# matajoh/fourier_feature_nets

Measured on AMD Instinct MI355X. Metric: rays/sec (train), higher is better.
Workload: dtype f32

## Files before the change

### fourier_feature_nets_amd/csrc/wgrad_common.h

```cpp
#pragma once
#include "common.h"

namespace ffn {

typedef float f32x4 __attribute__((ext_vector_type(4)));
typedef float f32x16 __attribute__((ext_vector_type(16)));

constexpr int kPartialFloats = 16 * 16 * 64 + 256;

__host__ __device__ __forceinline__ constexpr int ffn_wgrad_fold(int n_quads) {
    return n_quads <= 8 ? 4 : (n_quads <= 16 ? 2 : 1);
}

__device__ __forceinline__ f32x4 zero4() { f32x4 z; z[0] = z[1] = z[2] = z[3] = 0.0f; return z; }

template <typename T>
__device__ __forceinline__ T* uniform_ptr(T* p) {
    const uint64_t v = reinterpret_cast<uint64_t>(p);
    const uint32_t lo = __builtin_amdgcn_readfirstlane((uint32_t)v);
    const uint32_t hi = __builtin_amdgcn_readfirstlane((uint32_t)(v >> 32));
    return reinterpret_cast<T*>(((uint64_t)hi << 32) | lo);
}

constexpr int kImageBytes = 32 * 1024;
constexpr int kImageStride = kImageBytes + 512;
constexpr int kUnitLdsBytes = 4 * kImageStride;
__device__ __forceinline__ constexpr int image_a(int cur) { return cur * kImageStride; }
__device__ __forceinline__ constexpr int image_b(int cur) { return (2 + cur) * kImageStride; }

__device__ __forceinline__ void head_segment(const ffn_mlp_chain& ch, const ffn_wgrad_unit& unit,
                                             const ffn_wgrad_segment& seg, char* smem,
                                             const float* __restrict__ saved,
                                             const float* __restrict__ d_logits, int64_t n,
                                             int64_t num_blocks, float* __restrict__ partials) {
    const int tid = threadIdx.x;
    const int lane = tid & 63;
    const int sb = lane >> 2;
    const int li = lane & 3;
    const int wave = __builtin_amdgcn_readfirstlane(tid >> 6);
    const int lg_col = unit.m_slot, lg_n = unit.m_cq0;
    const bool col_ok = li < lg_n;
    const int64_t x_stride = (int64_t)ch.slot_channels[unit.n_slot] * 128;
    const char* x_s = reinterpret_cast<const char*>(saved + ch.slot_offset[unit.n_slot] * num_blocks * 32) +
                      unit.n_cq0 * 512 + seg.blk_begin * x_stride;
    x_s = uniform_ptr(x_s);
    const int c_last = (unit.n_quads >> 3) - 1;
    const int t16 = tid * 16;
    f32x4 acc[16];
#pragma unroll
    for (int q = 0; q < 16; ++q) acc[q] = zero4();
    float bsum = 0.0f;
    const int dl_lane = 4 * sb + (col_ok ? lg_col + li : 0);
    auto load_dl = [&](int64_t blk, float (&dst)[2]) {
        typedef const float __attribute__((address_space(1)))* gfloat;
        if ((blk + 1) * 32 <= n) {
            gfloat base = (gfloat)uniform_ptr(d_logits + blk * 128);
#pragma unroll
            for (int hs = 0; hs < 2; ++hs) {
                const float v = base[dl_lane + 64 * hs];
                dst[hs] = col_ok ? v : 0.0f;
            }
        } else {
#pragma unroll
            for (int hs = 0; hs < 2; ++hs) {
                const int64_t sample = blk * 32 + 16 * hs + sb;
                const int64_t sc = sample < n ? sample : n - 1;
                const float v = d_logits[sc * 4 + (col_ok ? lg_col + li : 0)];
                dst[hs] = (col_ok && sample < n) ? v : 0.0f;
            }
        }
    };
    f32x4 R[8];
    typedef const f32x4 __attribute__((address_space(1)))* gptr;
#define FFN_REQUEST(j)                                                                         \
    do {                                                                                       \
        gptr chunk = (gptr)(x_s + ((j) < c_last ? (j) : c_last) * 4096);                       \
        asm volatile("" : "+s"(chunk));                                                        \
        R[j] = __builtin_nontemporal_load(&chunk[tid]);                                                                     \
    } while (0)
#define FFN_DEPOSIT(cur, j) *reinterpret_cast<f32x4*>(smem + image_a(cur) + (j) * 4096 + t16) = R[j]
    float dl[2], dl_next[2];
    load_dl(seg.blk_begin, dl);
#pragma unroll
    for (int j = 0; j < 8; ++j) FFN_REQUEST(j);
#pragma unroll
    for (int j = 0; j < 8; ++j) FFN_DEPOSIT(0, j);
    x_s += x_stride;
    if (seg.blk_begin + 1 < seg.blk_end) {
#pragma unroll
        for (int j = 0; j < 8; ++j) FFN_REQUEST(j);
    }
    x_s += x_stride;
    asm volatile("s_waitcnt lgkmcnt(0)" ::: "memory");
    __builtin_amdgcn_s_barrier();
    unsigned a_at[16];
#pragma unroll
    for (int q = 0; q < 16; ++q) {
        const int quad = 16 * wave + q;
        a_at[q] = quad < unit.n_quads ? (unsigned)(quad * 512 + ((sb ^ q) << 4) + 4 * li)
                                      : (unsigned)(kImageBytes + 4 * li);
    }
    for (int64_t blk = seg.blk_begin; blk < seg.blk_end; ++blk) {
        const int cur = (int)((blk - seg.blk_begin) & 1);
        const bool has1 = blk + 1 < seg.blk_end, has2 = blk + 2 < seg.blk_end;
        load_dl(has1 ? blk + 1 : blk, dl_next);
        const char* img = smem + image_a(cur);
        bsum += dl[0] + dl[1];
#pragma unroll
        for (int q = 0; q < 16; ++q) {
            const float a0 = *reinterpret_cast<const float*>(img + a_at[q]);
            const float a1 = *reinterpret_cast<const float*>(img + a_at[q] + 256);
            acc[q] = __builtin_amdgcn_mfma_f32_4x4x1f32(a0, dl[0], acc[q], 0, 0, 0);
            acc[q] = __builtin_amdgcn_mfma_f32_4x4x1f32(a1, dl[1], acc[q], 0, 0, 0);
            if (q < 8) {
                if (q < 2) {
                    if (has1) {
#pragma unroll
                        for (int jj = 0; jj < 4; ++jj) FFN_DEPOSIT(cur ^ 1, q * 4 + jj);
                    }
                } else if (q < 6) {
                    if (has2) {
#pragma unroll
                        for (int jj = 0; jj < 2; ++jj) FFN_REQUEST((q - 2) * 2 + jj);
                    }
                }
            }
        }
        x_s += x_stride;
        asm volatile("s_waitcnt lgkmcnt(0)" ::: "memory");
        __builtin_amdgcn_s_barrier();
        dl[0] = dl_next[0];
        dl[1] = dl_next[1];
    }
#undef FFN_REQUEST
#undef FFN_DEPOSIT
    float* out = partials + (int64_t)(seg.slot + wave) * kPartialFloats;
#pragma unroll
    for (int q = 0; q < 16; ++q)
#pragma unroll
        for (int i = 0; i < 4; ++i) out[(q * 4 + i) * 64 + lane] = acc[q][i];
    out[16 * 16 * 64 + lane] = bsum;
}

}
```

### fourier_feature_nets_amd/mlp_engine.py

```python

import ctypes
import os
from typing import Dict, List, Optional, Sequence

import torch

from . import _lib
from ._lib import c_i, c_i64
from .ops import _call, _dev, _want, _want_numel

MAX_STEPS = 16
BIAS_LDS_FLOATS = 4096
WGRAD_GROUPS = 256
UNIT_COST = {4: 24, 2: 13, 1: 8}
HEAD_COST = 5
FOLD_COST = {(2, 2): 7, (2, 4): 5, (1, 2): 4, (1, 4): 3}
if os.environ.get("FFN_FOLD_COST"):
    _c = [int(v) for v in os.environ["FFN_FOLD_COST"].split(",")]
    FOLD_COST = {(2, 2): _c[0], (2, 4): _c[1], (1, 2): _c[2], (1, 4): _c[3]}
UNIT_COST16 = {4: 24, 2: 24, 1: 20}
HEAD_COST16 = 13
if os.environ.get("FFN_UNIT_COST16"):
    _c = [int(v) for v in os.environ["FFN_UNIT_COST16"].split(",")]
    UNIT_COST16, HEAD_COST16 = {4: _c[0], 2: _c[1], 1: _c[2]}, _c[3]
UNIT_COST_X6 = {4: 24, 2: 17, 1: 17}
HEAD_COST_X6 = 10
if os.environ.get("FFN_UNIT_COST_X6"):
    _c = [int(v) for v in os.environ["FFN_UNIT_COST_X6"].split(",")]
    UNIT_COST_X6, HEAD_COST_X6 = {4: _c[0], 2: _c[1], 1: _c[2]}, _c[3]
if os.environ.get("FFN_UNIT_COST"):
    _c = [int(v) for v in os.environ["FFN_UNIT_COST"].split(",")]
    UNIT_COST, HEAD_COST = {4: _c[0], 2: _c[1], 1: _c[2]}, _c[3]


TAIL_PAIRS = os.environ.get("FFN_TAIL_PAIRS", "1") == "1"
TAIL_QUADS = os.environ.get("FFN_TAIL_QUADS", "1") == "1"
TAIL_MAX_FULL_ROUNDS = 16


class FfnEncoding(ctypes.Structure):
    _fields_ = [("b", ctypes.c_void_p), ("a", ctypes.c_void_p), ("num_freq", ctypes.c_int32),
                ("include_input", ctypes.c_int32), ("scale", ctypes.c_float),
                ("width", ctypes.c_int32)]


class FfnStep(ctypes.Structure):
    _fields_ = [("act_groups", ctypes.c_int32), ("aux_groups", ctypes.c_int32),
                ("enc_id", ctypes.c_int32), ("lg_col", ctypes.c_int32), ("lg_n", ctypes.c_int32),
                ("out_tiles", ctypes.c_int32), ("relu", ctypes.c_int32), ("dst", ctypes.c_int32),
                ("out_col", ctypes.c_int32), ("out_n", ctypes.c_int32),
                ("save_in_slot", ctypes.c_int32), ("save_out_slot", ctypes.c_int32),
                ("mask_slot", ctypes.c_int32), ("save_enc_slot", ctypes.c_int32),
                ("head_off", ctypes.c_int32), ("out_slot", ctypes.c_int32),
                ("w_off", ctypes.c_int64), ("b_off", ctypes.c_int64)]


class FfnMlpChain(ctypes.Structure):
    _fields_ = [("enc", FfnEncoding * 2), ("step", FfnStep * MAX_STEPS),
                ("num_steps", ctypes.c_int32), ("num_slots", ctypes.c_int32),
                ("bias_floats", ctypes.c_int32), ("wide", ctypes.c_int32),
                ("slot_channels", ctypes.c_int32 * MAX_STEPS),
                ("slot_offset", ctypes.c_int64 * MAX_STEPS)]


class FfnWgradUnit(ctypes.Structure):
    _fields_ = [("m_slot", ctypes.c_int32), ("m_cq0", ctypes.c_int32), ("m_quads", ctypes.c_int32),
                ("want_bias", ctypes.c_int32), ("n_slot", ctypes.c_int32), ("n_cq0", ctypes.c_int32),
                ("n_quads", ctypes.c_int32), ("kind", ctypes.c_int32)]


class FfnWgradSegment(ctypes.Structure):
    _fields_ = [("job", ctypes.c_int32), ("slot", ctypes.c_int32),
                ("blk_begin", ctypes.c_int64), ("blk_end", ctypes.c_int64)]


class FfnReduceJob(ctypes.Structure):
    _fields_ = [("kind", ctypes.c_int32), ("slot_begin", ctypes.c_int32),
                ("slot_end", ctypes.c_int32), ("m_ch0", ctypes.c_int32), ("rows", ctypes.c_int32),
                ("n_quad0", ctypes.c_int32), ("n_quads", ctypes.c_int32),
                ("k_base", ctypes.c_int32), ("ld", ctypes.c_int32), ("has_bias", ctypes.c_int32),
                ("lg_n", ctypes.c_int32), ("slot_stride", ctypes.c_int32),
                ("n_fold", ctypes.c_int32), ("reserved", ctypes.c_int32),
                ("w_grad_off", ctypes.c_int64), ("b_grad_off", ctypes.c_int64),
                ("col_map", ctypes.c_void_p)]


class FfnPackJob(ctypes.Structure):
    _fields_ = [("src", ctypes.c_void_p), ("dst", ctypes.c_void_p), ("col_map", ctypes.c_void_p),
                ("kind", ctypes.c_int32), ("rows", ctypes.c_int32), ("cols", ctypes.c_int32),
                ("ld", ctypes.c_int32), ("transpose", ctypes.c_int32), ("groups", ctypes.c_int32),
                ("tiles", ctypes.c_int32), ("dst_rs", ctypes.c_int32), ("dst_cs", ctypes.c_int32),
                ("reserved", ctypes.c_int32)]


class FfnRenderRays(ctypes.Structure):
    _fields_ = [("starts", ctypes.c_void_p), ("directions", ctypes.c_void_p),
                ("near_far", ctypes.c_void_p), ("num_rays_total", ctypes.c_int64),
                ("ray_index", ctypes.c_void_p), ("ray_base", ctypes.c_int64),
                ("valid", ctypes.c_void_p), ("num_rays", ctypes.c_int32),
                ("num_samples", ctypes.c_int32), ("unit", ctypes.c_void_p),
                ("t_values", ctypes.c_void_p)]


class FfnOccupancy(ctypes.Structure):
    _fields_ = [("bits", ctypes.c_void_p), ("box_min", ctypes.c_float * 3),
                ("box_size", ctypes.c_float * 3), ("resolution", ctypes.c_int32)]


class FfnRenderOut(ctypes.Structure):
    _fields_ = [("color", ctypes.c_void_p), ("alpha", ctypes.c_void_p), ("depth", ctypes.c_void_p),
                ("nan_flag", ctypes.c_void_p), ("image", ctypes.c_void_p),
                ("pixel_offset", ctypes.c_int64)]


def _struct_array_to_device(items, device):
    if not items:
        return torch.zeros((0,), dtype=torch.uint8, device=device)
    arr = (type(items[0]) * len(items))(*items)
    host = torch.frombuffer(bytearray(bytes(arr)), dtype=torch.uint8)
    return host.to(device)


class EncodingSpec:

    def __init__(self, b: Optional[torch.Tensor], a: Optional[torch.Tensor], scale: float,
                 include_input: bool, device: Optional[torch.device] = None, num_inputs: int = 3):
        if num_inputs not in (1, 2, 3):
            raise NotImplementedError("encodings of 1, 2 or 3 inputs (got %d)" % num_inputs)
        self.num_inputs = int(num_inputs)
        self.num_freq = 0 if b is None else int(b.shape[1])
        dev = device if device is not None else (b.device if b is not None else None)
        if b is None:
            b = torch.zeros((3, 1), dtype=torch.float32, device=dev)
        elif b.shape[0] != num_inputs:
            raise ValueError("B has %d rows for %d inputs" % (b.shape[0], num_inputs))
        elif num_inputs < 3:
            b = torch.cat([b, torch.zeros((3 - num_inputs, b.shape[1]), dtype=b.dtype,
                                          device=b.device)])
        if a is None:
            a = torch.ones((max(self.num_freq, 1),), dtype=torch.float32, device=dev)
        self.b = b.contiguous()
        self.a = a.contiguous()
        self.scale = float(scale)
        self.include_input = bool(include_input) or self.num_freq == 0
        if self.num_freq > 256:
            raise NotImplementedError("encodings with more than 256 frequencies")
        natural = 2 * self.num_freq + (self.num_inputs if self.include_input else 0)
        self.natural_width = natural
        self.width = ((natural + 31) // 32) * 32

    def natural_index(self, internal: int) -> int:
        freq = self.num_freq
        if internal < 2 * freq:
            k = internal >> 1
            return k if (internal & 1) == 0 else freq + k
        if self.include_input and internal < 2 * freq + self.num_inputs:
            return internal
        return -1


class DenseSpec:

    def __init__(self, weight, bias, act_in: int, enc_id: Optional[int], relu: bool,
                 to_logits: Optional[tuple] = None):
        self.weight = weight
        self.bias = bias
        self.act_in = int(act_in)
        self.enc_id = enc_id
        self.relu = bool(relu)
        self.to_logits = to_logits
        self.out = int(weight.shape[0])
        self.ld = int(weight.shape[1])
        self.out_p = self.out
        self.act_in_p = self.act_in


MAX_HIDDEN_CHANNELS = 1024


def _padded_width(channels: int, wide=False) -> int:
    widths = {0: (32, 64, 128, 256), 1: (64, 128, 256, 512), 3: (128, 256, 512, 1024)}[int(wide)]
    for width in widths:
        if channels <= width:
            return width
    raise NotImplementedError("fused MLP kernels support hidden layers of up to %d channels "
                              "(got %d)" % (MAX_HIDDEN_CHANNELS, channels))


def _tiles(channels: int, wide=False) -> int:
    return _padded_width(channels, wide) // 32


class Workspace:

    def __init__(self, prog: "MlpProgram", n: int):
        self.n = n
        blocks = (n + 31) // 32
        self._dz_floats = prog.dz_channels * 32 * blocks
        self._prog, self._blocks = prog, blocks
        self._plans = {}
        self.partials = None
        self.use_plan("f32")

    @property
    def dz(self) -> torch.Tensor:
        return self._prog._dz_buffer(self._dz_floats)

    def use_plan(self, precision: str):
        plan = self._plans.get(precision)
        if plan is None:
            dev = self._prog.device
            raw = self._prog._plan_wgrad(self._blocks, precision)
            launches = [(kind, _struct_array_to_device(segs, dev), torch.tensor(starts, dtype=torch.int32, device=dev))
                        for kind, segs, starts in raw["launches"]]
            plan = dict(unit_segments=launches[0][1], unit_seg_start=launches[0][2], launches=launches,
                        reduce_jobs=_struct_array_to_device(raw["reduce_jobs"], dev),
                        num_reduce_jobs=len(raw["reduce_jobs"]),
                        partial_floats=raw["slots"] * self._prog.partial_floats)
            self._plans[precision] = plan
        self.unit_segments = plan["unit_segments"]
        self.unit_seg_start = plan["unit_seg_start"]
        self.launches = plan["launches"]
        self.reduce_jobs = plan["reduce_jobs"]
        self.num_reduce_jobs = plan["num_reduce_jobs"]
        if self.partials is None or self.partials.numel() < plan["partial_floats"]:
            self.partials = torch.empty((plan["partial_floats"],), dtype=torch.float32,
                                        device=self._prog.device)


class MlpProgram:

    def __init__(self, encodings: Sequence[EncodingSpec], layers: Sequence[DenseSpec],
                 device: torch.device, planning_only: bool = False):
        if device.type != "cuda" and not planning_only:
            raise RuntimeError("MlpProgram needs a GPU device; there is no CPU fallback")
        if len(layers) > MAX_STEPS:
            raise NotImplementedError("at most %d dense layers" % MAX_STEPS)
        self.partial_floats = 16 * 16 * 64 + 256
        if not planning_only:
            lib = _lib.load()
            lib.ffn_mlp_wgrad_partial_floats.restype = ctypes.c_int64
            assert int(lib.ffn_mlp_wgrad_partial_floats()) == self.partial_floats
        self.device = device
        self.encodings = list(encodings)
        self.layers = list(layers)
        self.uses_views = any(spec.enc_id == 1 for spec in self.layers)
        self._workspaces: Dict[int, Workspace] = {}
        self._build_forward()
        self._build_backward()
        self._build_wgrad_jobs()
        self._build_forward16()
        self._build_backward16()
        self._build_x6()
        self._build_pair_chains()

    def _dz_buffer(self, floats: int) -> torch.Tensor:
        buf = getattr(self, "_dz", None)
        if buf is None or buf.numel() < floats:
            self._dz = buf = None
            self._dz = buf = torch.empty((floats + floats // 16,), dtype=torch.float32,
                                         device=self.device)
        return buf[:floats]

    def release_workspaces(self):
        self._dz = None
        self._workspaces.clear()

    def _fill_encodings(self, chain):
        for i, enc in enumerate(self.encodings):
            e = chain.enc[i]
            e.b = enc.b.data_ptr()
            e.a = enc.a.data_ptr()
            e.num_freq = enc.num_freq
            e.include_input = 1 if enc.include_input else 0
            e.scale = enc.scale
            e.width = enc.width
        for i in range(len(self.encodings), 2):
            src = chain.enc[0]
            chain.enc[i].b, chain.enc[i].a = src.b, src.a
            chain.enc[i].num_freq, chain.enc[i].include_input = src.num_freq, src.include_input
            chain.enc[i].scale, chain.enc[i].width = src.scale, src.width

    def _build_forward(self):
        fwd = FfnMlpChain()
        self._fill_encodings(fwd)
        widest = max([sp.out for sp in self.layers if sp.to_logits is None] or [0])
        self.wide = widest > 256
        self.big = widest > 512
        self.wide_level = 3 if self.big else (1 if self.wide else 0)
        fwd.wide = self.wide_level
        producer = -1
        for i, sp in enumerate(self.layers):
            sp.act_in_p = self.layers[producer].out_p if (sp.act_in > 0 and producer >= 0) else sp.act_in
            if sp.to_logits is None:
                sp.out_p = _padded_width(sp.out, self.wide_level)
                producer = i
        w_off = b_off = h_off = 0
        self.col_maps: List[torch.Tensor] = []
        self.step_of: List[Optional[int]] = []
        self.fwd_shapes: Dict[int, tuple] = {}
        self.fused_heads = []
        self.grad_w_off, self.grad_b_off = [], []
        self.slot_of: Dict[int, int] = {}
        self.producer_of: List[int] = []
        slot_off = 0
        g_off = 0
        last_producer = -1
        stepped_consumers = set()
        prev = -1
        for j, sp in enumerate(self.layers):
            fusable = sp.to_logits is not None and sp.enc_id is None and sp.act_in > 0
            if sp.act_in > 0 and not fusable:
                stepped_consumers.add(prev)
            if sp.to_logits is None:
                prev = j
        num_steps = 0
        for i, spec in enumerate(self.layers):
            enc = None if spec.enc_id is None else self.encodings[spec.enc_id]
            self.producer_of.append(last_producer if spec.act_in > 0 else -1)
            if spec.act_in > 0 and (last_producer < 0 or
                                    self.layers[last_producer].out != spec.act_in):
                raise ValueError("layer %d consumes %d channels but the previous producer "
                                 "wrote a different width" % (i, spec.act_in))
            act_groups = spec.act_in_p // 8
            cmap = [c if c < spec.act_in else -1 for c in range(8 * act_groups)]
            if enc is not None:
                for c in range(enc.width):
                    nat = enc.natural_index(c)
                    cmap.append(-1 if nat < 0 else spec.act_in + nat)
# ... 813 lines not shown
```

Measured before the change: 1.544 million.

## Triple-buffer head wgrad loads and batch LDS reads with ds_read2st64

Restructures the head weight-gradient segment loop so that two register sets of global loads are kept in flight and the d_logits values are prefetched two blocks ahead. Each block's LDS operands are fetched up front with a single ds_read2st64 per quad, using the buffer toggle as an immediate offset, and the loop is unrolled by two so the current buffer is a compile-time constant. Deposits and requests are interleaved with the MFMA stream under explicit sched barriers. The scheduler's head cost constants are lowered to match the expected cheaper head segment. In exchange, register pressure rises from the doubled prefetch buffers, and the inline assembly ties the code to the LDS layout.

```diff
diff --git a/fourier_feature_nets_amd/csrc/wgrad_common.h b/fourier_feature_nets_amd/csrc/wgrad_common.h
--- a/fourier_feature_nets_amd/csrc/wgrad_common.h
+++ b/fourier_feature_nets_amd/csrc/wgrad_common.h
@@ -1,8 +1,11 @@
 #pragma once
+#include <type_traits>
+
 #include "common.h"
 
 namespace ffn {
 
+typedef float f32x2 __attribute__((ext_vector_type(2)));
 typedef float f32x4 __attribute__((ext_vector_type(4)));
 typedef float f32x16 __attribute__((ext_vector_type(16)));
 
@@ -51,89 +54,114 @@
     for (int q = 0; q < 16; ++q) acc[q] = zero4();
     float bsum = 0.0f;
     const int dl_lane = 4 * sb + (col_ok ? lg_col + li : 0);
-    auto load_dl = [&](int64_t blk, float (&dst)[2]) {
+    auto load_dl = [&](int64_t blk, float (&raw)[2]) {
         typedef const float __attribute__((address_space(1)))* gfloat;
         if ((blk + 1) * 32 <= n) {
             gfloat base = (gfloat)uniform_ptr(d_logits + blk * 128);
 #pragma unroll
-            for (int hs = 0; hs < 2; ++hs) {
-                const float v = base[dl_lane + 64 * hs];
-                dst[hs] = col_ok ? v : 0.0f;
-            }
+            for (int hs = 0; hs < 2; ++hs) raw[hs] = base[dl_lane + 64 * hs];
         } else {
 #pragma unroll
             for (int hs = 0; hs < 2; ++hs) {
                 const int64_t sample = blk * 32 + 16 * hs + sb;
                 const int64_t sc = sample < n ? sample : n - 1;
-                const float v = d_logits[sc * 4 + (col_ok ? lg_col + li : 0)];
-                dst[hs] = (col_ok && sample < n) ? v : 0.0f;
+                raw[hs] = d_logits[sc * 4 + (col_ok ? lg_col + li : 0)];
             }
         }
     };
-    f32x4 R[8];
+    auto mask_dl = [&](int64_t blk, const float (&raw)[2], float (&dst)[2]) {
+#pragma unroll
+        for (int hs = 0; hs < 2; ++hs) dst[hs] = (col_ok && blk * 32 + 16 * hs + sb < n) ? raw[hs] : 0.0f;
+    };
+    f32x4 R[2][8];
+    int64_t x_blk = seg.blk_begin;
     typedef const f32x4 __attribute__((address_space(1)))* gptr;
-#define FFN_REQUEST(j)                                                                         \
+#define FFN_REQUEST(set, j)                                                                    \
     do {                                                                                       \
         gptr chunk = (gptr)(x_s + ((j) < c_last ? (j) : c_last) * 4096);                       \
         asm volatile("" : "+s"(chunk));                                                        \
-        R[j] = __builtin_nontemporal_load(&chunk[tid]);                                                                     \
+        R[set][j] = __builtin_nontemporal_load(&chunk[tid]);                                   \
     } while (0)
-#define FFN_DEPOSIT(cur, j) *reinterpret_cast<f32x4*>(smem + image_a(cur) + (j) * 4096 + t16) = R[j]
-    float dl[2], dl_next[2];
-    load_dl(seg.blk_begin, dl);
+#define FFN_DEPOSIT(cur, set, j) *reinterpret_cast<f32x4*>(smem + image_a(cur) + (j) * 4096 + t16) = R[set][j]
+#define FFN_ADVANCE()                                                                          \
+    do {                                                                                       \
+        if (x_blk + 1 < seg.blk_end) {                                                         \
+            ++x_blk;                                                                           \
+            x_s += x_stride;                                                                   \
+        }                                                                                      \
+    } while (0)
+    float dl[2], dl_next[2], dl_raw[2][2];
+    auto dl_block = [&](int64_t blk) { return blk < seg.blk_end ? blk : seg.blk_end - 1; };
+    load_dl(seg.blk_begin, dl_raw[0]);
+    mask_dl(seg.blk_begin, dl_raw[0], dl);
 #pragma unroll
-    for (int j = 0; j < 8; ++j) FFN_REQUEST(j);
+    for (int j = 0; j < 8; ++j) FFN_REQUEST(0, j);
 #pragma unroll
-    for (int j = 0; j < 8; ++j) FFN_DEPOSIT(0, j);
-    x_s += x_stride;
-    if (seg.blk_begin + 1 < seg.blk_end) {
+    for (int j = 0; j < 8; ++j) FFN_DEPOSIT(0, 0, j);
+    FFN_ADVANCE();
 #pragma unroll
-        for (int j = 0; j < 8; ++j) FFN_REQUEST(j);
-    }
-    x_s += x_stride;
+    for (int j = 0; j < 8; ++j) FFN_REQUEST(1, j);
+    FFN_ADVANCE();
+#pragma unroll
+    for (int j = 0; j < 8; ++j) FFN_REQUEST(0, j);
+    FFN_ADVANCE();
+    load_dl(dl_block(seg.blk_begin + 1), dl_raw[0]);
+    load_dl(dl_block(seg.blk_begin + 2), dl_raw[1]);
     asm volatile("s_waitcnt lgkmcnt(0)" ::: "memory");
     __builtin_amdgcn_s_barrier();
+    const unsigned lds0 = (unsigned)(size_t)smem;
     unsigned a_at[16];
 #pragma unroll
     for (int q = 0; q < 16; ++q) {
         const int quad = 16 * wave + q;
-        a_at[q] = quad < unit.n_quads ? (unsigned)(quad * 512 + ((sb ^ q) << 4) + 4 * li)
-                                      : (unsigned)(kImageBytes + 4 * li);
+        a_at[q] = lds0 + (quad < unit.n_quads ? (unsigned)(quad * 512 + ((sb ^ q) << 4) + 4 * li)
+                                              : (unsigned)(kImageBytes + 4 * li));
     }
-    for (int64_t blk = seg.blk_begin; blk < seg.blk_end; ++blk) {
-        const int cur = (int)((blk - seg.blk_begin) & 1);
-        const bool has1 = blk + 1 < seg.blk_end, has2 = blk + 2 < seg.blk_end;
-        load_dl(has1 ? blk + 1 : blk, dl_next);
-        const char* img = smem + image_a(cur);
+    static_assert(kImageStride % 256 == 0 && kImageStride / 256 + 1 < 256, "the toggle rides in offset0/1");
+    auto block_body = [&](auto cur_tag, int64_t blk) {
+        constexpr int CUR = decltype(cur_tag)::value;
+        constexpr int kToggle = CUR * (kImageStride / 256);
+        const bool has1 = blk + 1 < seg.blk_end;
+        f32x2 a[16];
+#pragma unroll
+        for (int q = 0; q < 16; ++q)
+            asm volatile("ds_read2st64_b32 %0, %1 offset0:%2 offset1:%3"
+                         : "=v"(a[q]) : "v"(a_at[q]), "i"(kToggle), "i"(kToggle + 1) : "memory");
+        __builtin_amdgcn_sched_barrier(0);
+        if (has1) {
+#pragma unroll
+            for (int j = 0; j < 8; ++j) FFN_DEPOSIT(1 - CUR, 1 - CUR, j);
+        }
+        mask_dl(blk + 1, dl_raw[CUR], dl_next);
+        load_dl(dl_block(blk + 3), dl_raw[CUR]);
+        FFN_REQUEST(1 - CUR, 0);
+        FFN_REQUEST(1 - CUR, 1);
         bsum += dl[0] + dl[1];
+        __builtin_amdgcn_sched_barrier(0);
+        asm volatile("s_waitcnt lgkmcnt(0)" ::: "memory");
+        __builtin_amdgcn_sched_barrier(0);
 #pragma unroll
         for (int q = 0; q < 16; ++q) {
-            const float a0 = *reinterpret_cast<const float*>(img + a_at[q]);
-            const float a1 = *reinterpret_cast<const float*>(img + a_at[q] + 256);
-            acc[q] = __builtin_amdgcn_mfma_f32_4x4x1f32(a0, dl[0], acc[q], 0, 0, 0);
-            acc[q] = __builtin_amdgcn_mfma_f32_4x4x1f32(a1, dl[1], acc[q], 0, 0, 0);
-            if (q < 8) {
-                if (q < 2) {
-                    if (has1) {
+            acc[q] = __builtin_amdgcn_mfma_f32_4x4x1f32(a[q][0], dl[0], acc[q], 0, 0, 0);
+            if ((q & 1) && q < 12) FFN_REQUEST(1 - CUR, 2 + (q >> 1));
+        }
 #pragma unroll
-                        for (int jj = 0; jj < 4; ++jj) FFN_DEPOSIT(cur ^ 1, q * 4 + jj);
-                    }
-                } else if (q < 6) {
-                    if (has2) {
-#pragma unroll
-                        for (int jj = 0; jj < 2; ++jj) FFN_REQUEST((q - 2) * 2 + jj);
-                    }
-                }
-            }
-        }
-        x_s += x_stride;
-        asm volatile("s_waitcnt lgkmcnt(0)" ::: "memory");
+        for (int q = 0; q < 16; ++q)
+            acc[q] = __builtin_amdgcn_mfma_f32_4x4x1f32(a[q][1], dl[1], acc[q], 0, 0, 0);
+        FFN_ADVANCE();
         __builtin_amdgcn_s_barrier();
         dl[0] = dl_next[0];
         dl[1] = dl_next[1];
+    };
+    int64_t blk = seg.blk_begin;
+    for (; blk + 1 < seg.blk_end; blk += 2) {
+        block_body(std::integral_constant<int, 0>{}, blk);
+        block_body(std::integral_constant<int, 1>{}, blk + 1);
     }
+    if (blk < seg.blk_end) block_body(std::integral_constant<int, 0>{}, blk);
 #undef FFN_REQUEST
 #undef FFN_DEPOSIT
+#undef FFN_ADVANCE
     float* out = partials + (int64_t)(seg.slot + wave) * kPartialFloats;
 #pragma unroll
     for (int q = 0; q < 16; ++q)
diff --git a/fourier_feature_nets_amd/mlp_engine.py b/fourier_feature_nets_amd/mlp_engine.py
--- a/fourier_feature_nets_amd/mlp_engine.py
+++ b/fourier_feature_nets_amd/mlp_engine.py
@@ -13,18 +13,18 @@
 BIAS_LDS_FLOATS = 4096
 WGRAD_GROUPS = 256
 UNIT_COST = {4: 24, 2: 13, 1: 8}
-HEAD_COST = 5
+HEAD_COST = 3
 FOLD_COST = {(2, 2): 7, (2, 4): 5, (1, 2): 4, (1, 4): 3}
 if os.environ.get("FFN_FOLD_COST"):
     _c = [int(v) for v in os.environ["FFN_FOLD_COST"].split(",")]
     FOLD_COST = {(2, 2): _c[0], (2, 4): _c[1], (1, 2): _c[2], (1, 4): _c[3]}
 UNIT_COST16 = {4: 24, 2: 24, 1: 20}
-HEAD_COST16 = 13
+HEAD_COST16 = 8
 if os.environ.get("FFN_UNIT_COST16"):
     _c = [int(v) for v in os.environ["FFN_UNIT_COST16"].split(",")]
     UNIT_COST16, HEAD_COST16 = {4: _c[0], 2: _c[1], 1: _c[2]}, _c[3]
 UNIT_COST_X6 = {4: 24, 2: 17, 1: 17}
-HEAD_COST_X6 = 10
+HEAD_COST_X6 = 6
 if os.environ.get("FFN_UNIT_COST_X6"):
     _c = [int(v) for v in os.environ["FFN_UNIT_COST_X6"].split(",")]
     UNIT_COST_X6, HEAD_COST_X6 = {4: _c[0], 2: _c[1], 1: _c[2]}, _c[3]
```

New measurement: 1.548 million, median of 6. Within noise of the previous version (+0.3%).
